# sirpkt/flink-tensorflow

Measured on AMD Instinct MI355X. Metric: records/sec (whole node) + p50 per-record latency, ResNet-50 stream DP=1/8, higher is better.
Workload: dtype bf16

## Files before the change

### flink_tensorflow_amd/kernels/bottleneck.hip

```cpp
#include <pybind11/pybind11.h>

#include <cstdlib>
#include <stdexcept>
#include <string>
#include <type_traits>

#include "common.h"

namespace {

constexpr int CX = 64;
constexpr int CO = 256;
constexpr int NT = 512;

template <int CPR>
FTM_DEVICE int swz(int row, int c) {
  if constexpr (CPR == 8) return row * 8 + (c ^ ((row >> 1) & 7));
  else return row * CPR + (c ^ (row & 15));
}

template <int TP, int CN, bool DUAL>
__global__ __launch_bounds__(NT, 1) void bottleneck_tail_kernel(const bf16* __restrict__ x2, const bf16* __restrict__ xs,
                                                                const bf16* __restrict__ res,
                                                                const bf16* __restrict__ w3, const float* __restrict__ b3,
                                                                const bf16* __restrict__ w1, const float* __restrict__ b1,
                                                                bf16* __restrict__ y3, bf16* __restrict__ y1, int M,
                                                                int dec_h, int dec_w) {
  constexpr int CM = DUAL ? 2 * CX : CX;
  constexpr int W3_BYTES = CO * CM * 2;
  constexpr int W1_BYTES = CN * CO * 2;
  constexpr int X_BYTES = TP * (CN > CM ? CN : CM) * 2;
  constexpr int XCH = TP * CM / 8, OCH = TP * CN / 8, YCH = TP * CO / 8;
  constexpr int PF = TP / 16;
  constexpr int WPG = 8 / PF;
  constexpr int NF2 = CN / WPG / 16;
  static_assert(PF * WPG == 8 && NF2 >= 1 && XCH % NT == 0 && OCH % NT == 0 && YCH % NT == 0, "tile shape");
  extern __shared__ __attribute__((aligned(16))) uint8_t smem[];
  u32x4* W3s = reinterpret_cast<u32x4*>(smem);
  u32x4* W1s = reinterpret_cast<u32x4*>(smem + W3_BYTES);
  u32x4* Xs = reinterpret_cast<u32x4*>(smem + W3_BYTES + W1_BYTES);
  u32x4* Ys = reinterpret_cast<u32x4*>(smem + W3_BYTES + W1_BYTES + X_BYTES);
  const int tid = threadIdx.x, lane = tid & 63, wave = tid >> 6;
  const int prow = lane & 15, kg = lane >> 4;
  const int ntiles = (M + TP - 1) / TP;
  if ((int)blockIdx.x >= ntiles) return;

  constexpr int XC = CM / 8;
  for (int q = tid; q < CO * CM / 8; q += NT) W3s[swz<XC>(q / XC, q % XC)] = reinterpret_cast<const u32x4*>(w3)[q];
  for (int q = tid; q < CN * CO / 8; q += NT) W1s[swz<32>(q >> 5, q & 31)] = reinterpret_cast<const u32x4*>(w1)[q];

  constexpr int XIT = XCH / NT;
  u32x4 xr[XIT];
  auto load_x = [&](int t) {
#pragma unroll
    for (int it = 0; it < XIT; ++it) {
      const int q = tid + it * NT;
      const int px = t * TP + q / XC, c = q % XC;
      const bf16* srcp = (!DUAL || c < 8) ? x2 : xs;
      xr[it] = px < M ? reinterpret_cast<const u32x4*>(srcp + (size_t)px * CX)[c & 7] : u32x4{0u, 0u, 0u, 0u};
    }
  };
  auto store_x = [&]() {
#pragma unroll
    for (int it = 0; it < XIT; ++it) {
      const int q = tid + it * NT;
      Xs[swz<XC>(q / XC, q % XC)] = xr[it];
    }
  };

  constexpr int YIT = YCH / NT;
  static_assert(NT / (CO / 8) == 16, "pass: 16 pixels per iteration");
  u32x4 rv[YIT];
  auto load_r = [&](int tt) {
#pragma unroll
    for (int it = 0; it < YIT; ++it) {
      const int q = tid + it * NT;
      const int px = tt * TP + (q >> 5);
      rv[it] = (!DUAL && px < M) ? reinterpret_cast<const u32x4*>(res + (size_t)px * CO)[q & 31]
                                 : u32x4{0u, 0u, 0u, 0u};
    }
  };

  int t = blockIdx.x;
  load_r(t);
  load_x(t);
  store_x();
  __syncthreads();
  while (true) {
    const int p0 = t * TP;
    f32x4 acc[2][PF];
#pragma unroll
    for (int i = 0; i < 2; ++i)
#pragma unroll
      for (int j = 0; j < PF; ++j) acc[i][j] = f32x4{0.f, 0.f, 0.f, 0.f};
#pragma unroll
    for (int ks = 0; ks < CM / 32; ++ks) {
      const int c = ks * 4 + kg;
      bf16x8 a[2];
#pragma unroll
      for (int i = 0; i < 2; ++i) a[i] = __builtin_bit_cast(bf16x8, W3s[swz<XC>(wave * 32 + i * 16 + prow, c)]);
#pragma unroll
      for (int j = 0; j < PF; ++j) {
        const bf16x8 b = __builtin_bit_cast(bf16x8, Xs[swz<XC>(j * 16 + prow, c)]);
#pragma unroll
        for (int i = 0; i < 2; ++i) acc[i][j] = __builtin_amdgcn_mfma_f32_16x16x32_bf16(a[i], b, acc[i][j], 0, 0, 0);
      }
    }
#pragma unroll
    for (int i = 0; i < 2; ++i) {
      const int co = wave * 32 + i * 16 + kg * 4;
      const f32x4 bv = *reinterpret_cast<const f32x4*>(b3 + co);
#pragma unroll
      for (int j = 0; j < PF; ++j) {
        bf16x4 o;
#pragma unroll
        for (int r = 0; r < 4; ++r) o[r] = f2bf(acc[i][j][r] + bv[r]);
        const int px = j * 16 + prow;
        bf16* chunk = reinterpret_cast<bf16*>(Ys + swz<32>(px, co >> 3));
        *reinterpret_cast<bf16x4*>(chunk + (co & 7)) = o;
      }
    }
    __syncthreads();
    {
      int dn = 0, dh = 0, dw = 0;
      if (dec_w) {
        const int o0 = p0 + (tid >> 5);
        dw = o0 % dec_w;
        const int tt = o0 / dec_w;
        dh = tt % dec_h;
        dn = tt / dec_h;
      }
#pragma unroll
      for (int it = 0; it < YIT; ++it) {
        const int q = tid + it * NT;
        const int pl = q >> 5, c = q & 31;
        const int si = swz<32>(pl, c);
        bf16x8 v = __builtin_bit_cast(bf16x8, Ys[si]);
        const bf16x8 r = __builtin_bit_cast(bf16x8, rv[it]);
#pragma unroll
        for (int e = 0; e < 8; ++e) v[e] = f2bf(fmaxf((float)v[e] + (float)r[e], 0.f));
        Ys[si] = __builtin_bit_cast(u32x4, v);
        int o = p0 + pl;
        bool st = o < M;
        if (dec_w) {
          if (it) {
            dw += 16;
            while (dw >= dec_w) {
              dw -= dec_w;
              if (++dh == dec_h) { dh = 0; ++dn; }
            }
          }
          st = st && !((dh | dw) & 1);
          o = (dn * (dec_h >> 1) + (dh >> 1)) * (dec_w >> 1) + (dw >> 1);
        }
        if (st) reinterpret_cast<u32x4*>(y3 + (size_t)o * CO)[c] = __builtin_bit_cast(u32x4, v);
      }
    }
    const int tn = t + gridDim.x;
    const bool more = tn < ntiles;
    if (more) {
      load_x(tn);
      if constexpr (!DUAL) load_r(tn);
    }
    __syncthreads();
    const int pf = wave / WPG, cbase = (wave % WPG) * NF2 * 16;
    f32x4 acc2[NF2];
#pragma unroll
    for (int i = 0; i < NF2; ++i) acc2[i] = f32x4{0.f, 0.f, 0.f, 0.f};
#pragma unroll
    for (int ks = 0; ks < CO / 32; ++ks) {
      const int c = ks * 4 + kg;
      const bf16x8 b = __builtin_bit_cast(bf16x8, Ys[swz<32>(pf * 16 + prow, c)]);
#pragma unroll
      for (int i = 0; i < NF2; ++i) {
        const bf16x8 a = __builtin_bit_cast(bf16x8, W1s[swz<32>(cbase + i * 16 + prow, c)]);
        acc2[i] = __builtin_amdgcn_mfma_f32_16x16x32_bf16(a, b, acc2[i], 0, 0, 0);
      }
    }
#pragma unroll
    for (int i = 0; i < NF2; ++i) {
      const int co = cbase + i * 16 + kg * 4;
      const f32x4 bv = *reinterpret_cast<const f32x4*>(b1 + co);
      bf16x4 o;
#pragma unroll
      for (int r = 0; r < 4; ++r) o[r] = f2bf(fmaxf(acc2[i][r] + bv[r], 0.f));
      bf16* chunk = reinterpret_cast<bf16*>(Xs + swz<CN / 8>(pf * 16 + prow, co >> 3));
      *reinterpret_cast<bf16x4*>(chunk + (co & 7)) = o;
    }
    __syncthreads();
#pragma unroll
    for (int it = 0; it < OCH / NT; ++it) {
      const int q = tid + it * NT;
      const int pl = q / (CN / 8), c = q % (CN / 8);
      if (p0 + pl < M) reinterpret_cast<u32x4*>(y1 + (size_t)(p0 + pl) * CN)[c] = Xs[swz<CN / 8>(pl, c)];
    }
    if (!more) break;
    __syncthreads();
    store_x();
    __syncthreads();
    t = tn;
  }
}

template <int TP, int CN, bool DUAL>
void launch_tail(const bf16* x2, const bf16* xs, const bf16* res, const bf16* w3, const float* b3, const bf16* w1,
                 const float* b1, bf16* y3, bf16* y1, int M, int num_cu, hipStream_t stream, int dec_h, int dec_w) {
  constexpr int CM = DUAL ? 2 * CX : CX;
  const int tiles = (M + TP - 1) / TP;
  const int grid = tiles < num_cu ? tiles : num_cu;
  const size_t lds = CO * CM * 2 + CN * CO * 2 + TP * (CN > CM ? CN : CM) * 2 + TP * CO * 2;
  static_assert(CO * CM * 2 + CN * CO * 2 + TP * (CN > CM ? CN : CM) * 2 + TP * CO * 2 <= 160 * 1024, "LDS");
  hipFuncSetAttribute((const void*)bottleneck_tail_kernel<TP, CN, DUAL>, hipFuncAttributeMaxDynamicSharedMemorySize,
                      lds);
  hipLaunchKernelGGL((bottleneck_tail_kernel<TP, CN, DUAL>), dim3(grid), dim3(NT), lds, stream, x2, xs, res, w3, b3, w1,
                     b1, y3, y1, M, dec_h, dec_w);
}


}

void bottleneck_tail_bf16(uintptr_t x2, uintptr_t xs, uintptr_t res, uintptr_t w3, uintptr_t b3, uintptr_t w1,
                          uintptr_t b1, uintptr_t y3, uintptr_t y1, int M, int cn, int num_cu, uintptr_t stream,
                          int dec_h, int dec_w) {
  if (M <= 0) throw std::invalid_argument("bottleneck_tail: empty problem");
  if ((long)M * CO >= (1L << 31)) throw std::invalid_argument("bottleneck_tail: tensor too large for 32-bit indexing");
  const bool dual = xs != 0;
  if (dual == (res != 0)) throw std::invalid_argument("bottleneck_tail: pass exactly one of xs (dual) and res");
  for (uintptr_t p : {x2, dual ? xs : res, w3, w1, y3, y1, b3, b1})
    if (!p || p % 16) throw std::invalid_argument("bottleneck_tail: null or non-16-byte-aligned pointer");
  if (dec_w < 0 || dec_h < 0 || (dec_w > 0) != (dec_h > 0) || dec_w % 2 || dec_h % 2 ||
      (dec_w > 0 && M % (dec_h * dec_w)))
    throw std::invalid_argument("bottleneck_tail: decimation needs even H, W dividing the pixel count");
  auto s = reinterpret_cast<hipStream_t>(stream);
  auto bp = [](uintptr_t p) { return reinterpret_cast<bf16*>(p); };
  auto fp = [](uintptr_t p) { return reinterpret_cast<const float*>(p); };
  if (dual && cn == 64)
    launch_tail<64, 64, true>(bp(x2), bp(xs), nullptr, bp(w3), fp(b3), bp(w1), fp(b1), bp(y3), bp(y1), M, num_cu, s, dec_h, dec_w);
  else if (!dual && cn == 64)
    launch_tail<128, 64, false>(bp(x2), nullptr, bp(res), bp(w3), fp(b3), bp(w1), fp(b1), bp(y3), bp(y1), M, num_cu, s, dec_h, dec_w);
  else if (!dual && cn == 128)
    launch_tail<64, 128, false>(bp(x2), nullptr, bp(res), bp(w3), fp(b3), bp(w1), fp(b1), bp(y3), bp(y1), M, num_cu, s, dec_h, dec_w);
  else
    throw std::invalid_argument("bottleneck_tail: unsupported variant (dual " + std::to_string(dual) + ", cn " +
                                std::to_string(cn) + ")");
  FTM_CHECK_LAUNCH();
}

void register_bottleneck(pybind11::module_& m) {
  m.def("bottleneck_tail_bf16", &bottleneck_tail_bf16);
}
```

### flink_tensorflow_amd/kernels/bottleneck_chain.hip

```cpp
#include <pybind11/pybind11.h>

#include <stdexcept>
#include <string>

#include "common.h"

namespace {

constexpr int CX = 64;
constexpr int CO = 256;
constexpr int NT = 512;
constexpr int TP = 64;
constexpr int PF = TP / 16;

struct Link {
  const bf16* x;
  const bf16* xs;
  const bf16* w;
  const float* b;
};

struct ChainParams {
  Link l[3];
  const bf16* w1;
  const float* b1;
  bf16* y3;
  bf16* y1;
  int M, dec_h, dec_w;
};

template <int CPR>
FTM_DEVICE int swz(int row, int c) {
  if constexpr (CPR == 8) return row * 8 + (c ^ ((row >> 1) & 7));
  else return row * CPR + (c ^ (row & 15));
}

template <int J, int CN, bool STORE>
__global__ __launch_bounds__(NT, 1) void bottleneck_chain_kernel(ChainParams p) {
  constexpr int S = J + 1;
  constexpr int XS = TP * CX * 2;
  constexpr int XB = S * XS;
  constexpr int YB = TP * CO * 2;
  constexpr int CF = CN / 16;
  constexpr int WPC = 8 / CF;
  constexpr int PPW = PF / WPC;
  constexpr int PIECES = S * XS / 1024;
  static_assert(CF * WPC == 8 && PPW * WPC == PF && PIECES % 8 == 0, "tile split");
  extern __shared__ __attribute__((aligned(1024))) uint8_t smem[];
  u32x4* Ys = reinterpret_cast<u32x4*>(smem + 2 * XB);
  u32x4* Os = reinterpret_cast<u32x4*>(smem + 2 * XB + YB);
  const int tid = threadIdx.x, lane = tid & 63;
  const int wave = __builtin_amdgcn_readfirstlane(tid >> 6);
  const int prow = lane & 15, kg = lane >> 4;
  const int M = p.M;
  const int ntiles = (M + TP - 1) / TP;
  if ((int)blockIdx.x >= ntiles) return;

  bf16x8 wa0[2][4], wa1[2][2], wa2[2][2];
#pragma unroll
  for (int i = 0; i < 2; ++i) {
    const int co = wave * 32 + i * 16 + prow;
#pragma unroll
    for (int ks = 0; ks < 4; ++ks)
      wa0[i][ks] = *reinterpret_cast<const bf16x8*>(p.l[0].w + (size_t)co * 128 + ks * 32 + kg * 8);
    if constexpr (J >= 2)
#pragma unroll
      for (int ks = 0; ks < 2; ++ks)
        wa1[i][ks] = *reinterpret_cast<const bf16x8*>(p.l[1].w + (size_t)co * 64 + ks * 32 + kg * 8);
    if constexpr (J >= 3)
#pragma unroll
      for (int ks = 0; ks < 2; ++ks)
        wa2[i][ks] = *reinterpret_cast<const bf16x8*>(p.l[2].w + (size_t)co * 64 + ks * 32 + kg * 8);
  }
  const int cf = wave / WPC;
  const int pf0 = (wave % WPC) * PPW;
  bf16x8 wb[8];
#pragma unroll
  for (int ks = 0; ks < 8; ++ks)
    wb[ks] = *reinterpret_cast<const bf16x8*>(p.w1 + (size_t)(cf * 16 + prow) * CO + ks * 32 + kg * 8);

  const unsigned nbytes = (unsigned)M * CX * 2u;
  __amdgpu_buffer_rsrc_t rs[4];
#pragma unroll
  for (int sidx = 0; sidx < S; ++sidx) {
    const bf16* sp = sidx == 0 ? p.l[0].x : sidx == 1 ? p.l[0].xs : sidx == 2 ? p.l[1].x : p.l[2].x;
    rs[sidx] = __builtin_amdgcn_make_buffer_rsrc((void*)sp, 0, (int)nbytes, 0x00020000);
  }
  const int drow = lane >> 3, dslot = lane & 7;
  auto dma = [&](int t, int stage) {
#pragma unroll
    for (int k0 = 0; k0 < PIECES / 8; ++k0) {
      const int k = wave * (PIECES / 8) + k0;
      const int sidx = k >> 3, q = k & 7;
      const int row = q * 8 + drow;
      const int c = dslot ^ ((row >> 1) & 7);
      const unsigned off = (unsigned)(t * TP + row) * (CX * 2u) + (unsigned)c * 16u;
      uint8_t* dst = smem + stage * XB + sidx * XS + q * 1024;
      __builtin_amdgcn_raw_ptr_buffer_load_lds(rs[sidx], (__attribute__((address_space(3))) void*)dst, 16,
                                               (unsigned)(t * TP + row) < (unsigned)M ? off : 0x80000000u, 0, 0, 0);
    }
  };

  auto mma64 = [&](f32x4 (&acc)[2][PF / 2], const bf16x8 (&wa)[2][2], const u32x4* X, int j0) {
#pragma unroll
    for (int ks = 0; ks < 2; ++ks) {
      const int c = ks * 4 + kg;
#pragma unroll
      for (int j = 0; j < PF / 2; ++j) {
        const bf16x8 b = __builtin_bit_cast(bf16x8, X[swz<8>((j0 + j) * 16 + prow, c)]);
#pragma unroll
        for (int i = 0; i < 2; ++i) acc[i][j] = __builtin_amdgcn_mfma_f32_16x16x32_bf16(wa[i][ks], b, acc[i][j], 0, 0, 0);
      }
    }
  };
  auto finish = [&](f32x4 (&acc)[2][PF / 2], f32x4 (&res)[2][PF / 2], const float* b, bool first) {
#pragma unroll
    for (int i = 0; i < 2; ++i) {
      const f32x4 bv = *reinterpret_cast<const f32x4*>(b + wave * 32 + i * 16 + kg * 4);
#pragma unroll
      for (int j = 0; j < PF / 2; ++j)
#pragma unroll
        for (int r = 0; r < 4; ++r) {
          const float v = (float)f2bf(acc[i][j][r] + bv[r]);
          res[i][j][r] = (float)f2bf(fmaxf(first ? v : v + res[i][j][r], 0.f));
        }
    }
  };
  auto store_y1 = [&](int pt) {
#pragma unroll
    for (int it = 0; it < TP * CN / 8 / NT; ++it) {
      const int q = tid + it * NT;
      const int pl = q / (CN / 8), c = q % (CN / 8);
      if (pt * TP + pl < M) reinterpret_cast<u32x4*>(p.y1 + (size_t)(pt * TP + pl) * CN)[c] = Os[swz<CN / 8>(pl, c)];
    }
  };

  int t = blockIdx.x;
  int stage = 0;
  int prev = -1;
  dma(t, 0);
  while (true) {
    const int p0 = t * TP;
    asm volatile("s_waitcnt vmcnt(0) lgkmcnt(0)" ::: "memory");
    __syncthreads();
    if (prev >= 0) store_y1(prev);
    const int tn = t + gridDim.x;
    const bool more = tn < ntiles;
    if (more) dma(tn, stage ^ 1);
    const u32x4* X = reinterpret_cast<const u32x4*>(smem + stage * XB);
#pragma unroll
    for (int half = 0; half < 2; ++half) {
      constexpr int PH = PF / 2;
      f32x4 y[2][PH], acc[2][PH];
      auto zero = [&]() {
#pragma unroll
        for (int i = 0; i < 2; ++i)
#pragma unroll
          for (int j = 0; j < PH; ++j) acc[i][j] = f32x4{0.f, 0.f, 0.f, 0.f};
      };
      const int j0 = half * PH;
      zero();
      {
        const bf16x8 w0a[2][2] = {{wa0[0][0], wa0[0][1]}, {wa0[1][0], wa0[1][1]}};
        const bf16x8 w0b[2][2] = {{wa0[0][2], wa0[0][3]}, {wa0[1][2], wa0[1][3]}};
        mma64(acc, w0a, X, j0);
        mma64(acc, w0b, X + TP * 8, j0);
      }
      finish(acc, y, p.l[0].b, true);
      if constexpr (J >= 2) {
        zero();
        mma64(acc, wa1, X + 2 * TP * 8, j0);
        finish(acc, y, p.l[1].b, false);
      }
      if constexpr (J >= 3) {
        zero();
        mma64(acc, wa2, X + 3 * TP * 8, j0);
        finish(acc, y, p.l[2].b, false);
      }
#pragma unroll
      for (int i = 0; i < 2; ++i) {
        const int co = wave * 32 + i * 16 + kg * 4;
#pragma unroll
        for (int j = 0; j < PH; ++j) {
          bf16x4 o;
#pragma unroll
          for (int r = 0; r < 4; ++r) o[r] = f2bf(y[i][j][r]);
          bf16* chunk = reinterpret_cast<bf16*>(Ys + swz<32>((j0 + j) * 16 + prow, co >> 3));
          *reinterpret_cast<bf16x4*>(chunk + (co & 7)) = o;
        }
      }
    }
    __syncthreads();
    if constexpr (STORE) {
      int dn = 0, dh = 0, dw = 0;
      if (p.dec_w) {
        const int o0 = p0 + (tid >> 5);
        dw = o0 % p.dec_w;
        const int tt = o0 / p.dec_w;
        dh = tt % p.dec_h;
        dn = tt / p.dec_h;
      }
#pragma unroll
      for (int it = 0; it < TP * CO / 8 / NT; ++it) {
        const int q = tid + it * NT;
        const int pl = q >> 5, c = q & 31;
        int o = p0 + pl;
        bool st = o < M;
        if (p.dec_w) {
          if (it) {
            dw += 16;
            while (dw >= p.dec_w) {
              dw -= p.dec_w;
              if (++dh == p.dec_h) { dh = 0; ++dn; }
            }
          }
          st = st && !((dh | dw) & 1);
          o = (dn * (p.dec_h >> 1) + (dh >> 1)) * (p.dec_w >> 1) + (dw >> 1);
        }
        if (st) reinterpret_cast<u32x4*>(p.y3 + (size_t)o * CO)[c] = Ys[swz<32>(pl, c)];
      }
    }
    f32x4 acc2[PPW];
#pragma unroll
    for (int q = 0; q < PPW; ++q) acc2[q] = f32x4{0.f, 0.f, 0.f, 0.f};
#pragma unroll
    for (int ks = 0; ks < 8; ++ks) {
      const int c = ks * 4 + kg;
#pragma unroll
      for (int q = 0; q < PPW; ++q) {
        const bf16x8 b = __builtin_bit_cast(bf16x8, Ys[swz<32>((pf0 + q) * 16 + prow, c)]);
        acc2[q] = __builtin_amdgcn_mfma_f32_16x16x32_bf16(wb[ks], b, acc2[q], 0, 0, 0);
      }
    }
    {
      const int co = cf * 16 + kg * 4;
      const f32x4 bv = *reinterpret_cast<const f32x4*>(p.b1 + co);
#pragma unroll
      for (int q = 0; q < PPW; ++q) {
        bf16x4 o;
#pragma unroll
        for (int r = 0; r < 4; ++r) o[r] = f2bf(fmaxf(acc2[q][r] + bv[r], 0.f));
        bf16* chunk = reinterpret_cast<bf16*>(Os + swz<CN / 8>((pf0 + q) * 16 + prow, co >> 3));
        *reinterpret_cast<bf16x4*>(chunk + (co & 7)) = o;
      }
    }
    prev = t;
    if (!more) break;
    t = tn;
    stage ^= 1;
  }
  __syncthreads();
  store_y1(prev);
}

template <int J, int CN, bool STORE>
void launch_chain(const ChainParams& p, int num_cu, hipStream_t s) {
  constexpr int XB = (J + 1) * TP * CX * 2, YB = TP * CO * 2, OB = TP * CN * 2;
  constexpr int LDS = 2 * XB + YB + OB;
  static_assert(LDS <= 160 * 1024, "LDS");
  const int tiles = (p.M + TP - 1) / TP;
  const int grid = tiles < num_cu ? tiles : num_cu;
  hipFuncSetAttribute((const void*)bottleneck_chain_kernel<J, CN, STORE>, hipFuncAttributeMaxDynamicSharedMemorySize,
                      LDS);
  hipLaunchKernelGGL((bottleneck_chain_kernel<J, CN, STORE>), dim3(grid), dim3(NT), LDS, s, p);
}

template <int J>
void dispatch_cn(const ChainParams& p, int cn, bool store, int num_cu, hipStream_t s) {
  if (cn == 64) {
    if (store) launch_chain<J, 64, true>(p, num_cu, s);
    else launch_chain<J, 64, false>(p, num_cu, s);
  } else {
    if (store) launch_chain<J, 128, true>(p, num_cu, s);
    else launch_chain<J, 128, false>(p, num_cu, s);
  }
}

}

void bottleneck_chain_bf16(pybind11::list links, uintptr_t w1, uintptr_t b1, uintptr_t y3, uintptr_t y1, int M, int cn,
                           int num_cu, uintptr_t stream, int dec_h, int dec_w) {
  const int J = (int)pybind11::len(links);
  if (J < 1 || J > 3) throw std::invalid_argument("bottleneck_chain: 1 to 3 links");
  if (M <= 0 || (long)M * CO >= (1L << 31)) throw std::invalid_argument("bottleneck_chain: bad pixel count");
  if (cn != 64 && cn != 128) throw std::invalid_argument("bottleneck_chain: reduce width 64 or 128");
  ChainParams p{};
  for (int j = 0; j < J; ++j) {
    pybind11::tuple t = links[j].cast<pybind11::tuple>();
    if (t.size() != 4) throw std::invalid_argument("bottleneck_chain: link tuple (x, xs, w, b)");
    const uintptr_t x = t[0].cast<uintptr_t>(), xs = t[1].cast<uintptr_t>(), w = t[2].cast<uintptr_t>(),
                    b = t[3].cast<uintptr_t>();
    if ((j == 0) != (xs != 0)) throw std::invalid_argument("bottleneck_chain: link 0 dual, the others plain");
    for (uintptr_t q : {x, w, b})
      if (!q || q % 16) throw std::invalid_argument("bottleneck_chain: null or non-16-byte-aligned pointer");
    if (xs % 16) throw std::invalid_argument("bottleneck_chain: xs alignment");
    p.l[j] = Link{reinterpret_cast<const bf16*>(x), reinterpret_cast<const bf16*>(xs), reinterpret_cast<const bf16*>(w),
                  reinterpret_cast<const float*>(b)};
  }
  for (uintptr_t q : {w1, b1, y1})
    if (!q || q % 16) throw std::invalid_argument("bottleneck_chain: null or non-16-byte-aligned pointer");
  if (y3 % 16) throw std::invalid_argument("bottleneck_chain: y3 alignment");
  if (dec_w < 0 || dec_h < 0 || (dec_w > 0) != (dec_h > 0) || dec_w % 2 || dec_h % 2 ||
      (dec_w > 0 && M % (dec_h * dec_w)))
    throw std::invalid_argument("bottleneck_chain: decimation needs even H, W dividing the pixel count");
  if (dec_w && !y3) throw std::invalid_argument("bottleneck_chain: decimation without y3");
  p.w1 = reinterpret_cast<const bf16*>(w1);
  p.b1 = reinterpret_cast<const float*>(b1);
  p.y3 = reinterpret_cast<bf16*>(y3);
  p.y1 = reinterpret_cast<bf16*>(y1);
  p.M = M;
  p.dec_h = dec_h;
  p.dec_w = dec_w;
  auto s = reinterpret_cast<hipStream_t>(stream);
  const bool store = y3 != 0;
  if (J == 1) dispatch_cn<1>(p, cn, store, num_cu, s);
  else if (J == 2) dispatch_cn<2>(p, cn, store, num_cu, s);
  else dispatch_cn<3>(p, cn, store, num_cu, s);
  FTM_CHECK_LAUNCH();
}

void register_bottleneck_chain(pybind11::module_& m) { m.def("bottleneck_chain_bf16", &bottleneck_chain_bf16); }
```

Baseline: 80120.

## Restructure bottleneck tail kernel with register weights, double-buffered LDS, software-pipelined MFMA

The tail kernel no longer stages W3 and W1 in LDS. Each wave now loads its weight fragments and biases into registers once. The X tile is double-buffered in LDS, and the y1 store for the previous tile is deferred into the next iteration. Global accesses switch to buffer loads and stores with an out-of-range offset to drop masked lanes. The LDS reads feeding the MFMAs are software-pipelined with sched_barriers in both kernels, and the chain kernel interleaves links with bias preloading. These changes aim to cut LDS traffic and barriers and to overlap LDS reads with MFMA work, at the cost of higher register pressure.

```diff
diff --git a/flink_tensorflow_amd/kernels/bottleneck.hip b/flink_tensorflow_amd/kernels/bottleneck.hip
--- a/flink_tensorflow_amd/kernels/bottleneck.hip
+++ b/flink_tensorflow_amd/kernels/bottleneck.hip
@@ -17,6 +17,12 @@
 FTM_DEVICE int swz(int row, int c) {
   if constexpr (CPR == 8) return row * 8 + (c ^ ((row >> 1) & 7));
   else return row * CPR + (c ^ (row & 15));
+}
+
+template <int TP, int CN, bool DUAL>
+constexpr int tail_lds_bytes() {
+  constexpr int CM = DUAL ? 2 * CX : CX;
+  return 2 * TP * CM * 2 + TP * CN * 2 + TP * CO * 2;
 }
 
 template <int TP, int CN, bool DUAL>
@@ -27,27 +33,54 @@
                                                                 bf16* __restrict__ y3, bf16* __restrict__ y1, int M,
                                                                 int dec_h, int dec_w) {
   constexpr int CM = DUAL ? 2 * CX : CX;
-  constexpr int W3_BYTES = CO * CM * 2;
-  constexpr int W1_BYTES = CN * CO * 2;
-  constexpr int X_BYTES = TP * (CN > CM ? CN : CM) * 2;
+  constexpr int KS1 = CM / 32;
+  constexpr int KS2 = CO / 32;
+  constexpr int XB = TP * CM * 2;
+  constexpr int OB = TP * CN * 2;
   constexpr int XCH = TP * CM / 8, OCH = TP * CN / 8, YCH = TP * CO / 8;
   constexpr int PF = TP / 16;
-  constexpr int WPG = 8 / PF;
-  constexpr int NF2 = CN / WPG / 16;
-  static_assert(PF * WPG == 8 && NF2 >= 1 && XCH % NT == 0 && OCH % NT == 0 && YCH % NT == 0, "tile shape");
+  constexpr int G1 = PF > 4 ? 2 : 4;
+  constexpr int NG = PF / G1;
+  constexpr int CF = CN / 16;
+  constexpr int WPC = 8 / CF;
+  constexpr int PPW = PF / WPC;
+  static_assert(CF * WPC == 8 && PPW * WPC == PF && NG * G1 == PF && XCH % NT == 0 && OCH % NT == 0 && YCH % NT == 0,
+                "tile shape");
   extern __shared__ __attribute__((aligned(16))) uint8_t smem[];
-  u32x4* W3s = reinterpret_cast<u32x4*>(smem);
-  u32x4* W1s = reinterpret_cast<u32x4*>(smem + W3_BYTES);
-  u32x4* Xs = reinterpret_cast<u32x4*>(smem + W3_BYTES + W1_BYTES);
-  u32x4* Ys = reinterpret_cast<u32x4*>(smem + W3_BYTES + W1_BYTES + X_BYTES);
-  const int tid = threadIdx.x, lane = tid & 63, wave = tid >> 6;
+  u32x4* Os = reinterpret_cast<u32x4*>(smem + 2 * XB);
+  u32x4* Ys = reinterpret_cast<u32x4*>(smem + 2 * XB + OB);
+  const int tid = threadIdx.x, lane = tid & 63;
+  const int wave = __builtin_amdgcn_readfirstlane(tid >> 6);
   const int prow = lane & 15, kg = lane >> 4;
   const int ntiles = (M + TP - 1) / TP;
   if ((int)blockIdx.x >= ntiles) return;
 
   constexpr int XC = CM / 8;
-  for (int q = tid; q < CO * CM / 8; q += NT) W3s[swz<XC>(q / XC, q % XC)] = reinterpret_cast<const u32x4*>(w3)[q];
-  for (int q = tid; q < CN * CO / 8; q += NT) W1s[swz<32>(q >> 5, q & 31)] = reinterpret_cast<const u32x4*>(w1)[q];
+  bf16x8 wa[2][KS1], wb[KS2];
+  f32x4 bv3[2];
+#pragma unroll
+  for (int i = 0; i < 2; ++i) {
+    const int co = wave * 32 + i * 16;
+#pragma unroll
+    for (int ks = 0; ks < KS1; ++ks)
+      wa[i][ks] = *reinterpret_cast<const bf16x8*>(w3 + (size_t)(co + prow) * CM + ks * 32 + kg * 8);
+    bv3[i] = *reinterpret_cast<const f32x4*>(b3 + co + kg * 4);
+  }
+  const int cf = wave / WPC;
+  const int pf0 = (wave % WPC) * PPW;
+#pragma unroll
+  for (int ks = 0; ks < KS2; ++ks)
+    wb[ks] = *reinterpret_cast<const bf16x8*>(w1 + (size_t)(cf * 16 + prow) * CO + ks * 32 + kg * 8);
+  const f32x4 bv1 = *reinterpret_cast<const f32x4*>(b1 + cf * 16 + kg * 4);
+
+  auto rsrc = [](const void* ptr, unsigned bytes) {
+    return __builtin_amdgcn_make_buffer_rsrc(const_cast<void*>(ptr), 0, (int)bytes, 0x00020000);
+  };
+  constexpr unsigned DROP = 0xFFFFFF00u;
+  const unsigned y3rows = dec_w ? (unsigned)M / 4u : (unsigned)M;
+  const __amdgpu_buffer_rsrc_t rx2 = rsrc(x2, (unsigned)M * CX * 2u), rxs = rsrc(DUAL ? xs : x2, (unsigned)M * CX * 2u);
+  const __amdgpu_buffer_rsrc_t rres = rsrc(DUAL ? (const bf16*)y3 : res, (unsigned)M * CO * 2u);
+  const __amdgpu_buffer_rsrc_t ry3 = rsrc(y3, y3rows * CO * 2u), ry1 = rsrc(y1, (unsigned)M * CN * 2u);
 
   constexpr int XIT = XCH / NT;
   u32x4 xr[XIT];
@@ -55,61 +88,90 @@
 #pragma unroll
     for (int it = 0; it < XIT; ++it) {
       const int q = tid + it * NT;
-      const int px = t * TP + q / XC, c = q % XC;
-      const bf16* srcp = (!DUAL || c < 8) ? x2 : xs;
-      xr[it] = px < M ? reinterpret_cast<const u32x4*>(srcp + (size_t)px * CX)[c & 7] : u32x4{0u, 0u, 0u, 0u};
-    }
-  };
-  auto store_x = [&]() {
+      const unsigned px = (unsigned)(t * TP + q / XC), c = q % XC;
+      const unsigned off = px < (unsigned)M ? px * (CX * 2u) + (c & 7) * 16u : DROP;
+      xr[it] = __builtin_amdgcn_raw_buffer_load_b128((DUAL && c >= 8) ? rxs : rx2, off, 0, 0);
+    }
+  };
+  auto store_x = [&](int stage) {
+    u32x4* Xn = reinterpret_cast<u32x4*>(smem + stage * XB);
 #pragma unroll
     for (int it = 0; it < XIT; ++it) {
       const int q = tid + it * NT;
-      Xs[swz<XC>(q / XC, q % XC)] = xr[it];
+      Xn[swz<XC>(q / XC, q % XC)] = xr[it];
+    }
+  };
+  auto store_y1 = [&](int pt) {
+#pragma unroll
+    for (int it = 0; it < OCH / NT; ++it) {
+      const int q = tid + it * NT;
+      const int pl = q / (CN / 8), c = q % (CN / 8);
+      const unsigned px = (unsigned)(pt * TP + pl);
+      __builtin_amdgcn_raw_buffer_store_b128(Os[swz<CN / 8>(pl, c)], ry1,
+                                             pt >= 0 && px < (unsigned)M ? px * (CN * 2u) + c * 16u : DROP, 0, 0);
     }
   };
 
   constexpr int YIT = YCH / NT;
-  static_assert(NT / (CO / 8) == 16, "pass: 16 pixels per iteration");
+  constexpr int YG = 4;
+  static_assert(NT / (CO / 8) == 16 && YIT % YG == 0, "pass: 16 pixels per iteration, groups of YG");
   u32x4 rv[YIT];
   auto load_r = [&](int tt) {
 #pragma unroll
     for (int it = 0; it < YIT; ++it) {
       const int q = tid + it * NT;
-      const int px = tt * TP + (q >> 5);
-      rv[it] = (!DUAL && px < M) ? reinterpret_cast<const u32x4*>(res + (size_t)px * CO)[q & 31]
-                                 : u32x4{0u, 0u, 0u, 0u};
-    }
-  };
-
+      const unsigned px = (unsigned)(tt * TP + (q >> 5));
+      if constexpr (DUAL) rv[it] = u32x4{0u, 0u, 0u, 0u};
+      else rv[it] = __builtin_amdgcn_raw_buffer_load_b128(rres, px < (unsigned)M ? px * (CO * 2u) + (q & 31) * 16u : DROP, 0, 0);
+    }
+  };
+
+  const int nwg = gridDim.x;
   int t = blockIdx.x;
+  int stage = 0;
+  int prev = -1;
   load_r(t);
   load_x(t);
-  store_x();
-  __syncthreads();
+  store_x(0);
   while (true) {
     const int p0 = t * TP;
+    asm volatile("s_waitcnt lgkmcnt(0)" ::: "memory");
+    __syncthreads();
+    store_y1(prev);
+    const int tn = t + nwg;
+    const bool more = tn < ntiles;
+    load_x(tn);
+    const u32x4* Xs = reinterpret_cast<const u32x4*>(smem + stage * XB);
     f32x4 acc[2][PF];
 #pragma unroll
     for (int i = 0; i < 2; ++i)
 #pragma unroll
       for (int j = 0; j < PF; ++j) acc[i][j] = f32x4{0.f, 0.f, 0.f, 0.f};
-#pragma unroll
-    for (int ks = 0; ks < CM / 32; ++ks) {
-      const int c = ks * 4 + kg;
-      bf16x8 a[2];
-#pragma unroll
-      for (int i = 0; i < 2; ++i) a[i] = __builtin_bit_cast(bf16x8, W3s[swz<XC>(wave * 32 + i * 16 + prow, c)]);
-#pragma unroll
-      for (int j = 0; j < PF; ++j) {
-        const bf16x8 b = __builtin_bit_cast(bf16x8, Xs[swz<XC>(j * 16 + prow, c)]);
-#pragma unroll
-        for (int i = 0; i < 2; ++i) acc[i][j] = __builtin_amdgcn_mfma_f32_16x16x32_bf16(a[i], b, acc[i][j], 0, 0, 0);
+    {
+      bf16x8 xb[2][G1];
+      auto read_x = [&](int s, bf16x8(&dst)[G1]) {
+        const int c = (s / NG) * 4 + kg, j0 = (s % NG) * G1;
+#pragma unroll
+        for (int g = 0; g < G1; ++g) dst[g] = __builtin_bit_cast(bf16x8, Xs[swz<XC>((j0 + g) * 16 + prow, c)]);
+      };
+      read_x(0, xb[0]);
+#pragma unroll
+      for (int s = 0; s < KS1 * NG; ++s) {
+        if (s + 1 < KS1 * NG) read_x(s + 1, xb[(s + 1) & 1]);
+        __builtin_amdgcn_sched_barrier(0);
+        const int ks = s / NG, j0 = (s % NG) * G1;
+#pragma unroll
+        for (int g = 0; g < G1; ++g)
+#pragma unroll
+          for (int i = 0; i < 2; ++i)
+            acc[i][j0 + g] = __builtin_amdgcn_mfma_f32_16x16x32_bf16(wa[i][ks], xb[s & 1][g], acc[i][j0 + g], 0, 0, 0);
+        __builtin_amdgcn_sched_barrier(0);
       }
     }
 #pragma unroll
     for (int i = 0; i < 2; ++i) {
       const int co = wave * 32 + i * 16 + kg * 4;
-      const f32x4 bv = *reinterpret_cast<const f32x4*>(b3 + co);
+      const f32x4 bv = bv3[i];
 #pragma unroll
       for (int j = 0; j < PF; ++j) {
         bf16x4 o;
@@ -130,12 +192,21 @@
         dh = tt % dec_h;
         dn = tt / dec_h;
       }
+      bf16x8 yv[YG];
 #pragma unroll
       for (int it = 0; it < YIT; ++it) {
+        if (it % YG == 0) {
+#pragma unroll
+          for (int g = 0; g < YG; ++g) {
+            const int q = tid + (it + g) * NT;
+            yv[g] = __builtin_bit_cast(bf16x8, Ys[swz<32>(q >> 5, q & 31)]);
+          }
+          __builtin_amdgcn_sched_barrier(0);
+        }
         const int q = tid + it * NT;
         const int pl = q >> 5, c = q & 31;
         const int si = swz<32>(pl, c);
-        bf16x8 v = __builtin_bit_cast(bf16x8, Ys[si]);
+        bf16x8 v = yv[it % YG];
         const bf16x8 r = __builtin_bit_cast(bf16x8, rv[it]);
 #pragma unroll
         for (int e = 0; e < 8; ++e) v[e] = f2bf(fmaxf((float)v[e] + (float)r[e], 0.f));
@@ -153,63 +224,59 @@
           st = st && !((dh | dw) & 1);
           o = (dn * (dec_h >> 1) + (dh >> 1)) * (dec_w >> 1) + (dw >> 1);
         }
-        if (st) reinterpret_cast<u32x4*>(y3 + (size_t)o * CO)[c] = __builtin_bit_cast(u32x4, v);
-      }
-    }
-    const int tn = t + gridDim.x;
-    const bool more = tn < ntiles;
-    if (more) {
-      load_x(tn);
-      if constexpr (!DUAL) load_r(tn);
-    }
+        __builtin_amdgcn_raw_buffer_store_b128(__builtin_bit_cast(u32x4, v), ry3,
+                                               st ? (unsigned)o * (CO * 2u) + c * 16u : DROP, 0, 0);
+      }
+    }
+    if constexpr (!DUAL) load_r(tn);
     __syncthreads();
-    const int pf = wave / WPG, cbase = (wave % WPG) * NF2 * 16;
-    f32x4 acc2[NF2];
-#pragma unroll
-    for (int i = 0; i < NF2; ++i) acc2[i] = f32x4{0.f, 0.f, 0.f, 0.f};
-#pragma unroll
-    for (int ks = 0; ks < CO / 32; ++ks) {
-      const int c = ks * 4 + kg;
-      const bf16x8 b = __builtin_bit_cast(bf16x8, Ys[swz<32>(pf * 16 + prow, c)]);
-#pragma unroll
-      for (int i = 0; i < NF2; ++i) {
-        const bf16x8 a = __builtin_bit_cast(bf16x8, W1s[swz<32>(cbase + i * 16 + prow, c)]);
-        acc2[i] = __builtin_amdgcn_mfma_f32_16x16x32_bf16(a, b, acc2[i], 0, 0, 0);
-      }
-    }
-#pragma unroll
-    for (int i = 0; i < NF2; ++i) {
-      const int co = cbase + i * 16 + kg * 4;
-      const f32x4 bv = *reinterpret_cast<const f32x4*>(b1 + co);
-      bf16x4 o;
-#pragma unroll
-      for (int r = 0; r < 4; ++r) o[r] = f2bf(fmaxf(acc2[i][r] + bv[r], 0.f));
-      bf16* chunk = reinterpret_cast<bf16*>(Xs + swz<CN / 8>(pf * 16 + prow, co >> 3));
-      *reinterpret_cast<bf16x4*>(chunk + (co & 7)) = o;
-    }
-    __syncthreads();
-#pragma unroll
-    for (int it = 0; it < OCH / NT; ++it) {
-      const int q = tid + it * NT;
-      const int pl = q / (CN / 8), c = q % (CN / 8);
-      if (p0 + pl < M) reinterpret_cast<u32x4*>(y1 + (size_t)(p0 + pl) * CN)[c] = Xs[swz<CN / 8>(pl, c)];
-    }
+    f32x4 acc2[PPW];
+#pragma unroll
+    for (int q = 0; q < PPW; ++q) acc2[q] = f32x4{0.f, 0.f, 0.f, 0.f};
+    {
+      bf16x8 yb[2][PPW];
+      auto read_y = [&](int ks, bf16x8(&dst)[PPW]) {
+#pragma unroll
+        for (int q = 0; q < PPW; ++q) dst[q] = __builtin_bit_cast(bf16x8, Ys[swz<32>((pf0 + q) * 16 + prow, ks * 4 + kg)]);
+      };
+      read_y(0, yb[0]);
+#pragma unroll
+      for (int ks = 0; ks < KS2; ++ks) {
+        if (ks + 1 < KS2) read_y(ks + 1, yb[(ks + 1) & 1]);
+        __builtin_amdgcn_sched_barrier(0);
+#pragma unroll
+        for (int q = 0; q < PPW; ++q) acc2[q] = __builtin_amdgcn_mfma_f32_16x16x32_bf16(wb[ks], yb[ks & 1][q], acc2[q], 0, 0, 0);
+        __builtin_amdgcn_sched_barrier(0);
+      }
+    }
+    {
+      const int co = cf * 16 + kg * 4;
+#pragma unroll
+      for (int q = 0; q < PPW; ++q) {
+        bf16x4 o;
+#pragma unroll
+        for (int r = 0; r < 4; ++r) o[r] = f2bf(fmaxf(acc2[q][r] + bv1[r], 0.f));
+        bf16* chunk = reinterpret_cast<bf16*>(Os + swz<CN / 8>((pf0 + q) * 16 + prow, co >> 3));
+        *reinterpret_cast<bf16x4*>(chunk + (co & 7)) = o;
+      }
+    }
+    prev = t;
     if (!more) break;
-    __syncthreads();
-    store_x();
-    __syncthreads();
+    store_x(stage ^ 1);
     t = tn;
+    stage ^= 1;
   }
+  __syncthreads();
+  store_y1(prev);
 }
 
 template <int TP, int CN, bool DUAL>
 void launch_tail(const bf16* x2, const bf16* xs, const bf16* res, const bf16* w3, const float* b3, const bf16* w1,
                  const float* b1, bf16* y3, bf16* y1, int M, int num_cu, hipStream_t stream, int dec_h, int dec_w) {
-  constexpr int CM = DUAL ? 2 * CX : CX;
   const int tiles = (M + TP - 1) / TP;
   const int grid = tiles < num_cu ? tiles : num_cu;
-  const size_t lds = CO * CM * 2 + CN * CO * 2 + TP * (CN > CM ? CN : CM) * 2 + TP * CO * 2;
-  static_assert(CO * CM * 2 + CN * CO * 2 + TP * (CN > CM ? CN : CM) * 2 + TP * CO * 2 <= 160 * 1024, "LDS");
+  constexpr size_t lds = tail_lds_bytes<TP, CN, DUAL>();
+  static_assert(lds <= 160 * 1024, "LDS");
   hipFuncSetAttribute((const void*)bottleneck_tail_kernel<TP, CN, DUAL>, hipFuncAttributeMaxDynamicSharedMemorySize,
                       lds);
   hipLaunchKernelGGL((bottleneck_tail_kernel<TP, CN, DUAL>), dim3(grid), dim3(NT), lds, stream, x2, xs, res, w3, b3, w1,
diff --git a/flink_tensorflow_amd/kernels/bottleneck_chain.hip b/flink_tensorflow_amd/kernels/bottleneck_chain.hip
--- a/flink_tensorflow_amd/kernels/bottleneck_chain.hip
+++ b/flink_tensorflow_amd/kernels/bottleneck_chain.hip
@@ -78,6 +78,12 @@
 #pragma unroll
   for (int ks = 0; ks < 8; ++ks)
     wb[ks] = *reinterpret_cast<const bf16x8*>(p.w1 + (size_t)(cf * 16 + prow) * CO + ks * 32 + kg * 8);
+  f32x4 bl[J][2];
+#pragma unroll
+  for (int j = 0; j < J; ++j)
+#pragma unroll
+    for (int i = 0; i < 2; ++i) bl[j][i] = *reinterpret_cast<const f32x4*>(p.l[j].b + wave * 32 + i * 16 + kg * 4);
+  const f32x4 bv1 = *reinterpret_cast<const f32x4*>(p.b1 + cf * 16 + kg * 4);
 
   const unsigned nbytes = (unsigned)M * CX * 2u;
   __amdgpu_buffer_rsrc_t rs[4];
@@ -101,30 +107,33 @@
     }
   };
 
-  auto mma64 = [&](f32x4 (&acc)[2][PF / 2], const bf16x8 (&wa)[2][2], const u32x4* X, int j0) {
-#pragma unroll
-    for (int ks = 0; ks < 2; ++ks) {
-      const int c = ks * 4 + kg;
-#pragma unroll
-      for (int j = 0; j < PF / 2; ++j) {
-        const bf16x8 b = __builtin_bit_cast(bf16x8, X[swz<8>((j0 + j) * 16 + prow, c)]);
-#pragma unroll
-        for (int i = 0; i < 2; ++i) acc[i][j] = __builtin_amdgcn_mfma_f32_16x16x32_bf16(wa[i][ks], b, acc[i][j], 0, 0, 0);
-      }
-    }
-  };
-  auto finish = [&](f32x4 (&acc)[2][PF / 2], f32x4 (&res)[2][PF / 2], const float* b, bool first) {
-#pragma unroll
-    for (int i = 0; i < 2; ++i) {
-      const f32x4 bv = *reinterpret_cast<const f32x4*>(b + wave * 32 + i * 16 + kg * 4);
-#pragma unroll
-      for (int j = 0; j < PF / 2; ++j)
+  constexpr int PH = PF / 2;
+  auto read_src = [&](bf16x8 (&dst)[2][PH], const u32x4* X, int src, int j0) {
+#pragma unroll
+    for (int ks = 0; ks < 2; ++ks)
+#pragma unroll
+      for (int j = 0; j < PH; ++j)
+        dst[ks][j] = __builtin_bit_cast(bf16x8, X[src * TP * 8 + swz<8>((j0 + j) * 16 + prow, ks * 4 + kg)]);
+  };
+  auto mma64 = [&](f32x4 (&acc)[2][PH], const bf16x8 (&w0)[2], const bf16x8 (&w1)[2], const bf16x8 (&xb)[2][PH]) {
+#pragma unroll
+    for (int ks = 0; ks < 2; ++ks)
+#pragma unroll
+      for (int j = 0; j < PH; ++j) {
+        acc[0][j] = __builtin_amdgcn_mfma_f32_16x16x32_bf16(w0[ks], xb[ks][j], acc[0][j], 0, 0, 0);
+        acc[1][j] = __builtin_amdgcn_mfma_f32_16x16x32_bf16(w1[ks], xb[ks][j], acc[1][j], 0, 0, 0);
+      }
+  };
+  auto finish = [&](const f32x4 (&acc)[2][PH], f32x4 (&res)[2][PH], const f32x4 (&bv)[2], bool first) {
+#pragma unroll
+    for (int i = 0; i < 2; ++i)
+#pragma unroll
+      for (int j = 0; j < PH; ++j)
 #pragma unroll
         for (int r = 0; r < 4; ++r) {
-          const float v = (float)f2bf(acc[i][j][r] + bv[r]);
+          const float v = (float)f2bf(acc[i][j][r] + bv[i][r]);
           res[i][j][r] = (float)f2bf(fmaxf(first ? v : v + res[i][j][r], 0.f));
         }
-    }
   };
   auto store_y1 = [&](int pt) {
 #pragma unroll
@@ -135,6 +144,7 @@
     }
   };
 
+  const int nwg = gridDim.x;
   int t = blockIdx.x;
   int stage = 0;
   int prev = -1;
@@ -144,51 +154,54 @@
     asm volatile("s_waitcnt vmcnt(0) lgkmcnt(0)" ::: "memory");
     __syncthreads();
     if (prev >= 0) store_y1(prev);
-    const int tn = t + gridDim.x;
+    const int tn = t + nwg;
     const bool more = tn < ntiles;
     if (more) dma(tn, stage ^ 1);
     const u32x4* X = reinterpret_cast<const u32x4*>(smem + stage * XB);
-#pragma unroll
-    for (int half = 0; half < 2; ++half) {
-      constexpr int PH = PF / 2;
-      f32x4 y[2][PH], acc[2][PH];
-      auto zero = [&]() {
-#pragma unroll
-        for (int i = 0; i < 2; ++i)
-#pragma unroll
-          for (int j = 0; j < PH; ++j) acc[i][j] = f32x4{0.f, 0.f, 0.f, 0.f};
+    {
+      constexpr int NST = 2 * S;
+      f32x4 y[2][PH], acc[2][2][PH];
+      bf16x8 xb[2][2][PH];
+      auto complete = [&](int half, int link, int a) {
+        finish(acc[a], y, bl[link], link == 0);
+        if (link == J - 1) {
+#pragma unroll
+          for (int i = 0; i < 2; ++i) {
+            const int co = wave * 32 + i * 16 + kg * 4;
+#pragma unroll
+            for (int j = 0; j < PH; ++j) {
+              bf16x4 o;
+#pragma unroll
+              for (int r = 0; r < 4; ++r) o[r] = f2bf(y[i][j][r]);
+              bf16* chunk = reinterpret_cast<bf16*>(Ys + swz<32>((half * PH + j) * 16 + prow, co >> 3));
+              *reinterpret_cast<bf16x4*>(chunk + (co & 7)) = o;
+            }
+          }
+        }
       };
-      const int j0 = half * PH;
-      zero();
-      {
-        const bf16x8 w0a[2][2] = {{wa0[0][0], wa0[0][1]}, {wa0[1][0], wa0[1][1]}};
-        const bf16x8 w0b[2][2] = {{wa0[0][2], wa0[0][3]}, {wa0[1][2], wa0[1][3]}};
-        mma64(acc, w0a, X, j0);
-        mma64(acc, w0b, X + TP * 8, j0);
-      }
-      finish(acc, y, p.l[0].b, true);
-      if constexpr (J >= 2) {
-        zero();
-        mma64(acc, wa1, X + 2 * TP * 8, j0);
-        finish(acc, y, p.l[1].b, false);
-      }
-      if constexpr (J >= 3) {
-        zero();
-        mma64(acc, wa2, X + 3 * TP * 8, j0);
-        finish(acc, y, p.l[2].b, false);
-      }
-#pragma unroll
-      for (int i = 0; i < 2; ++i) {
-        const int co = wave * 32 + i * 16 + kg * 4;
-#pragma unroll
-        for (int j = 0; j < PH; ++j) {
-          bf16x4 o;
-#pragma unroll
-          for (int r = 0; r < 4; ++r) o[r] = f2bf(y[i][j][r]);
-          bf16* chunk = reinterpret_cast<bf16*>(Ys + swz<32>((j0 + j) * 16 + prow, co >> 3));
-          *reinterpret_cast<bf16x4*>(chunk + (co & 7)) = o;
-        }
-      }
+      read_src(xb[0], X, 0, 0);
+#pragma unroll
+      for (int st = 0; st < NST; ++st) {
+        const int half = st / S, src = st % S;
+        const int link = src < 2 ? 0 : src - 1;
+        const int a = (half * J + link) & 1;
+        if (st + 1 < NST) read_src(xb[(st + 1) & 1], X, (st + 1) % S, ((st + 1) / S) * PH);
+        if (src != 1) {
+#pragma unroll
+          for (int i = 0; i < 2; ++i)
+#pragma unroll
+            for (int j = 0; j < PH; ++j) acc[a][i][j] = f32x4{0.f, 0.f, 0.f, 0.f};
+        }
+        if (src == 0) mma64(acc[a], {wa0[0][0], wa0[0][1]}, {wa0[1][0], wa0[1][1]}, xb[st & 1]);
+        else if (src == 1) mma64(acc[a], {wa0[0][2], wa0[0][3]}, {wa0[1][2], wa0[1][3]}, xb[st & 1]);
+        else if (src == 2) mma64(acc[a], wa1[0], wa1[1], xb[st & 1]);
+        else mma64(acc[a], wa2[0], wa2[1], xb[st & 1]);
+        if (st > 0 && (st - 1) % S != 0) {
+          const int ph = (st - 1) / S, pl = (st - 1) % S - 1;
+          complete(ph, pl, (ph * J + pl) & 1);
+        }
+      }
+      complete(1, J - 1, (J + J - 1) & 1);
     }
     __syncthreads();
     if constexpr (STORE) {
@@ -200,8 +213,16 @@
         dh = tt % p.dec_h;
         dn = tt / p.dec_h;
       }
-#pragma unroll
-      for (int it = 0; it < TP * CO / 8 / NT; ++it) {
+      constexpr int YIT = TP * CO / 8 / NT;
+      u32x4 yv[YIT];
+#pragma unroll
+      for (int it = 0; it < YIT; ++it) {
+        const int q = tid + it * NT;
+        yv[it] = Ys[swz<32>(q >> 5, q & 31)];
+      }
+      __builtin_amdgcn_sched_barrier(0);
+#pragma unroll
+      for (int it = 0; it < YIT; ++it) {
         const int q = tid + it * NT;
         const int pl = q >> 5, c = q & 31;
         int o = p0 + pl;
@@ -217,29 +238,35 @@
           st = st && !((dh | dw) & 1);
           o = (dn * (p.dec_h >> 1) + (dh >> 1)) * (p.dec_w >> 1) + (dw >> 1);
         }
-        if (st) reinterpret_cast<u32x4*>(p.y3 + (size_t)o * CO)[c] = Ys[swz<32>(pl, c)];
+        if (st) reinterpret_cast<u32x4*>(p.y3 + (size_t)o * CO)[c] = yv[it];
       }
     }
     f32x4 acc2[PPW];
 #pragma unroll
     for (int q = 0; q < PPW; ++q) acc2[q] = f32x4{0.f, 0.f, 0.f, 0.f};
-#pragma unroll
-    for (int ks = 0; ks < 8; ++ks) {
-      const int c = ks * 4 + kg;
-#pragma unroll
-      for (int q = 0; q < PPW; ++q) {
-        const bf16x8 b = __builtin_bit_cast(bf16x8, Ys[swz<32>((pf0 + q) * 16 + prow, c)]);
-        acc2[q] = __builtin_amdgcn_mfma_f32_16x16x32_bf16(wb[ks], b, acc2[q], 0, 0, 0);
+    {
+      bf16x8 yb[2][PPW];
+      auto read_y = [&](int ks, bf16x8 (&dst)[PPW]) {
+#pragma unroll
+        for (int q = 0; q < PPW; ++q) dst[q] = __builtin_bit_cast(bf16x8, Ys[swz<32>((pf0 + q) * 16 + prow, ks * 4 + kg)]);
+      };
+      read_y(0, yb[0]);
+#pragma unroll
+      for (int ks = 0; ks < 8; ++ks) {
+        if (ks + 1 < 8) read_y(ks + 1, yb[(ks + 1) & 1]);
+        __builtin_amdgcn_sched_barrier(0);
+#pragma unroll
+        for (int q = 0; q < PPW; ++q) acc2[q] = __builtin_amdgcn_mfma_f32_16x16x32_bf16(wb[ks], yb[ks & 1][q], acc2[q], 0, 0, 0);
+        __builtin_amdgcn_sched_barrier(0);
       }
     }
     {
       const int co = cf * 16 + kg * 4;
-      const f32x4 bv = *reinterpret_cast<const f32x4*>(p.b1 + co);
 #pragma unroll
       for (int q = 0; q < PPW; ++q) {
         bf16x4 o;
 #pragma unroll
-        for (int r = 0; r < 4; ++r) o[r] = f2bf(fmaxf(acc2[q][r] + bv[r], 0.f));
+        for (int r = 0; r < 4; ++r) o[r] = f2bf(fmaxf(acc2[q][r] + bv1[r], 0.f));
         bf16* chunk = reinterpret_cast<bf16*>(Os + swz<CN / 8>((pf0 + q) * 16 + prow, co >> 3));
         *reinterpret_cast<bf16x4*>(chunk + (co & 7)) = o;
       }
diff --git a/profiles/r07_tail_sched/isa_pattern.py b/profiles/r07_tail_sched/isa_pattern.py
--- /dev/null
+++ b/profiles/r07_tail_sched/isa_pattern.py
@@ -0,0 +1,24 @@
+import re, sys
+path, key = sys.argv[1], sys.argv[2]
+cur = None; out = []; valu = 0
+def flush():
+    global valu
+    if valu: out.append(f"V{valu}"); valu = 0
+for line in open(path):
+    m = re.match(r"^[0-9a-f]+ <(.+)>:", line)
+    if m: cur = m.group(1); continue
+    if cur is None or key not in cur: continue
+    t = line.strip().split("//")[0].split()
+    if not t: continue
+    op = t[0]
+    if op.startswith("v_mfma"): flush(); out.append("M")
+    elif op.startswith("ds_read"): flush(); out.append("R")
+    elif op.startswith("ds_write"): flush(); out.append("W")
+    elif op == "s_waitcnt": flush(); out.append("[" + "".join(t[1:]) + "]")
+    elif op == "s_barrier": flush(); out.append("\n==BAR==\n")
+    elif op.startswith("global_load") or op.startswith("buffer_load"): flush(); out.append("GL" if "lds" not in line else "DMA")
+    elif op.startswith("global_store") or op.startswith("buffer_store"): flush(); out.append("GS")
+    elif op.startswith("s_cbranch") or op.startswith("s_branch"): flush(); out.append("<" + op[2:] + ">")
+    elif op.startswith("v_"): valu += 1
+flush()
+print(" ".join(out))
```

After: 81920, median of 6. +2.3%, better.
